# ksahlin/IsoCon

Measured on AMD Instinct MI355X. Metric: read x candidate alignments/sec (NN-graph build, 50k x 2.5kb reads), higher is better.
Workload: dtype u64; 1 GPU; C3: 50000 synthetic CCS reads (50000 unique), ~2500 bp, 10 isoforms, seed 30001; 1-set NN graph; edges=78526, graph_digest=65944c838d76a6c9, parallelism=single GPU

## Files before the change

isocon_amd/csrc/nn_list.hpp:

```cpp
#pragma once
#include "nn.hpp"
#include "nn_surv_core.hpp"

namespace isocon {

static constexpr uint32_t NN_LIST_MIN = 256;
#ifndef ISOCON_NN_LIST_CHUNK
#define ISOCON_NN_LIST_CHUNK 2048
#endif
static constexpr uint32_t NN_LIST_CHUNK = ISOCON_NN_LIST_CHUNK;
static constexpr int NN_STAGE = NN_LIST_CHUNK + 64;
#ifndef ISOCON_SURV_WAVES
#define ISOCON_SURV_WAVES 1
#endif
static constexpr int NN_SURV_WAVES = ISOCON_SURV_WAVES;

struct NNPlanTotals {
    unsigned long long n_pairs, pad0[15], n_list, pad1[15], n_small, pad2[15], n_chunks, pad3[15], n_filtered, pad4[15], overflow, pad5[15];
    unsigned long long n_chunks_narrow, pad6[15];
    unsigned long long n_wide_pairs, n_narrow_listed, pad7[14];
    unsigned long long f_next, pad8[15], f_chunks, pad9[15], f_chunks_narrow, pad10[15], f_rejected, f_narrow_listed, f_listed, f_rejected2, pad11[12];
    unsigned long long f_tasks, pad12[15], f_task_next, pad13[15];
    unsigned long long n_seed_known, pad14[15];
};

static constexpr uint32_t NN_KNOWN_SLOTS = 8;
struct NNSeedKnown { const uint32_t *known; uint32_t drop; };
typedef uint32_t NNKnownRow __attribute__((ext_vector_type(4)));
__device__ __forceinline__ bool nn_seed_known(const uint32_t *__restrict__ known, uint32_t a, uint32_t b)
{
    const NNKnownRow *ra = reinterpret_cast<const NNKnownRow *>(known + (size_t)a * NN_KNOWN_SLOTS), *rb = reinterpret_cast<const NNKnownRow *>(known + (size_t)b * NN_KNOWN_SLOTS);
    const NNKnownRow a0 = ra[0], a1 = ra[1], b0 = rb[0], b1 = rb[1];
    bool hit = false;
#pragma unroll
    for (int i = 0; i < 4; ++i) hit = hit || a0[i] == b || a1[i] == b || b0[i] == a || b1[i] == a;
    return hit;
}

static constexpr int32_t NN_NARROW_K = 31;

struct NNBoundRows {
    const uint8_t *lb;  const unsigned long long *row_off; const uint32_t *row_len;
    const uint8_t *lbT; const unsigned long long *offT;    const uint32_t *sloT; const uint32_t *lenT;
    const uint32_t *score;
};

__device__ __forceinline__ uint32_t nn_meta_len(uint32_t w) { return w & 0x3fffu; }
__device__ __forceinline__ int32_t nn_meta_thr(uint32_t w) { return (int32_t)((w >> 14) & 0x7fu); }
__device__ __forceinline__ uint32_t nn_meta_score(uint32_t w) { return w >> 23; }
static constexpr uint32_t NN_META_PAD = 3;
typedef uint32_t NNMeta4 __attribute__((ext_vector_type(4), aligned(4)));

__global__ __launch_bounds__(256) void k_nn_entry_meta(DevStore S, NNParams P, const uint32_t *__restrict__ score, uint32_t *__restrict__ meta, NNPlanTotals *__restrict__ totals)
{
    const uint32_t x = blockIdx.x * 256u + threadIdx.x;
    if (x >= S.n && x < S.n + NN_META_PAD) meta[x] = 0u;
    if (x < S.n) {
        const int32_t m = S.lens[x], b = load_relaxed_agent(P.best + x);
        int32_t thr = b < m ? b : m;
        thr = thr < 64 ? thr : 64;
        const uint32_t sc = score[x] >> 5;
        const bool isq = P.qflag[x] != 0;
        meta[x] = ((uint32_t)m & 0x3fffu) | ((uint32_t)thr << 14) | ((P.tflag[x] != 0 ? 1u : 0u) << 21) | ((isq ? 1u : 0u) << 22) | ((sc < 511u ? sc : 511u) << 23);
    }
}

__global__ __launch_bounds__(64 * NN_SURV_WAVES) void k_nn_survivors(DevStore S, NNParams P, NNBoundRows B, const uint32_t *__restrict__ meta, QMap Q, uint32_t nq,
                                                       uint32_t *__restrict__ list, unsigned long long list_cap, NNChunk *__restrict__ chunks, unsigned long long chunks_cap,
                                                       uint32_t *__restrict__ pa, uint32_t *__restrict__ pb, unsigned long long small_cap, NNPlanTotals *__restrict__ totals, uint32_t list_min,
                                                       int32_t class_mode, NNSeedKnown K)
{
    __shared__ uint32_t stage[NN_SURV_WAVES][NN_STAGE];
    __shared__ uint32_t s_small[NN_SURV_WAVES], s_filtered[NN_SURV_WAVES], s_kept[NN_SURV_WAVES], s_known[NN_SURV_WAVES];
    __shared__ unsigned long long s_base;
    const int wave = threadIdx.x >> 6;
    const uint32_t x = blockIdx.x * (uint32_t)NN_SURV_WAVES + (uint32_t)wave;
    const int lane = threadIdx.x & 63;
    const uint32_t mx = x < S.n ? meta[x] : 0u;
    const bool x_isq = (mx & (1u << 22)) != 0, x_ist = (mx & (1u << 21)) != 0;
    uint32_t up_len = 0, dn_len = 0, dn_slo = 0;
    unsigned long long up_off = 0, dn_off = 0;
    if (x < S.n && (x_isq || x_ist)) {
        uint32_t s;
        if (Q.slot_of(x, s) && s < nq) {
            up_len = B.row_len[s];
            up_off = B.row_off[s];
        }
        dn_len = B.lenT[x]; dn_slo = B.sloT[x]; dn_off = B.offT[x];
    }
    const int32_t m = (int32_t)nn_meta_len(mx);
    const int32_t kx0 = nn_meta_thr(mx);
    const uint32_t sx = nn_meta_score(mx);
    uint32_t *st = stage[wave];
    uint32_t fill = 0, fill_n = 0, filtered = 0, kept = 0;
    auto emit_chunk = [&](bool narrow_class, bool merged = false) {
        const uint32_t cnt = merged ? fill + fill_n : narrow_class ? fill_n : fill;
        unsigned long long base = 0, ci = 0;
        if (lane == 0) {
            base = atomicAdd(&totals->n_list, (unsigned long long)cnt);
            ci = atomicAdd(narrow_class ? &totals->n_chunks_narrow : &totals->n_chunks, 1ull);
            if (narrow_class) atomicAdd(&totals->n_narrow_listed, (unsigned long long)cnt);
        }
        base = ((unsigned long long)(uint32_t)__builtin_amdgcn_readfirstlane((int)(base >> 32)) << 32) | (uint32_t)__builtin_amdgcn_readfirstlane((int)(uint32_t)base);
        ci = ((unsigned long long)(uint32_t)__builtin_amdgcn_readfirstlane((int)(ci >> 32)) << 32) | (uint32_t)__builtin_amdgcn_readfirstlane((int)(uint32_t)ci);
        if (base + cnt <= list_cap && ci < chunks_cap) {
            if (narrow_class) { for (uint32_t i = (uint32_t)lane; i < cnt; i += 64) list[base + i] = st[NN_STAGE - 1 - i]; }
            else { for (uint32_t i = (uint32_t)lane; i < cnt; i += 64) list[base + i] = i < fill ? st[i] : st[NN_STAGE - 1 - (i - fill)]; }
            if (lane == 0) { NNChunk ch; ch.slot = x; ch.count = cnt; ch.begin = base; chunks[(narrow_class ? chunks_cap : 0ull) + ci] = ch; }
        } else if (lane == 0) atomicOr(&totals->overflow, 1ull);
        if (narrow_class || merged) fill_n = 0;
        if (!narrow_class) fill = 0;
    };
#ifndef ISOCON_SURV_U
#define ISOCON_SURV_U 4
#endif
    constexpr int U = ISOCON_SURV_U;
    const uint32_t q_block = Q.block();
    const uint32_t role_mask = (x_isq ? 1u << 21 : 0u) | (x_ist ? 1u << 22 : 0u);
    auto entry_of = [&](uint32_t s) { return Q.begin + (s >> Q.block_log2) * Q.stride + (s & (q_block - 1u)); };
    auto scan_side = [&](auto side_tag) {
        constexpr int side = decltype(side_tag)::value;
        const uint32_t len = side == 0 ? up_len : dn_len;
        const uint8_t *row = side == 0 ? B.lb + up_off : B.lbT + dn_off;
        const uint32_t tail = (len - 1u) & ~3u;
        auto load_batches = [&](uint32_t c0, uint32_t (&lbv)[U], NNMeta4 (&my)[U]) {
#pragma unroll
            for (int u = 0; u < U; ++u) {
                const uint32_t e0 = c0 + (uint32_t)SURV_BATCH * u + 4u * (uint32_t)lane;
                const uint32_t ec = e0 < len ? e0 : tail;
                __builtin_memcpy(&lbv[u], row + ec, 4);
                if (side == 0) my[u] = *reinterpret_cast<const NNMeta4 *>(meta + (x + 1u + ec));
                else {
                    const uint32_t s0 = dn_slo + ec;
                    const bool apart = Q.stride != q_block && (s0 & (q_block - 1u)) + 3u >= q_block;
                    if (__builtin_amdgcn_ballot_w64(apart) == 0) my[u] = *reinterpret_cast<const NNMeta4 *>(meta + entry_of(s0));
                    else {
#pragma unroll
                        for (int b = 0; b < SURV_PER_LANE; ++b) my[u][b] = meta[entry_of(dn_slo + (ec + b < len ? ec + b : len - 1u))];
                    }
                }
            }
        };
        auto scan_batches = [&](uint32_t c0, const uint32_t (&lbv)[U], const NNMeta4 (&my)[U]) {
#pragma unroll
            for (int u = 0; u < U; ++u) {
                if (c0 + (uint32_t)SURV_BATCH * u >= len) break;
                const uint32_t e0 = c0 + (uint32_t)SURV_BATCH * u + 4u * (uint32_t)lane;
                uint64_t am[SURV_PER_LANE], an[SURV_PER_LANE], aw[SURV_PER_LANE];
#pragma unroll
                for (int b = 0; b < SURV_PER_LANE; ++b) {
                    const uint32_t myb = my[u][b];
                    const bool inr = e0 + b < len;
                    const bool xq = inr && x_isq && (myb & (1u << 21));
                    const bool yq = inr && x_ist && (myb & (1u << 22));
                    int32_t kx = -1, ky = -1;
                    if (xq) kx = kx0;
                    if (yq) ky = nn_meta_thr(myb);
                    int32_t k = kx > ky ? kx : ky;
                    if (k > P.kcap) k = P.kcap;
                    const int32_t dl = m - (int32_t)nn_meta_len(myb), ad = dl < 0 ? -dl : dl;
                    const uint32_t sy_u = nn_meta_score(myb);
                    const bool cand = inr && k >= 0 && ad <= k;
                    const bool accept = cand && (int32_t)((lbv[u] >> (8 * b)) & 0xffu) <= k;
                    const bool mine = accept && (side == 0 ? sy_u <= sx : sx > sy_u);
                    if (side == 0) { filtered += cand && !accept ? 1u : 0u; kept += accept ? 1u : 0u; }
                    const bool wide = mine && class_mode > 0 && k > NN_NARROW_K;
                    const bool keep = mine && !wide;
                    const bool to_narrow = keep && class_mode >= 0 && k <= NN_NARROW_K;
                    aw[b] = __builtin_amdgcn_ballot_w64(wide);
                    am[b] = __builtin_amdgcn_ballot_w64(keep && !to_narrow);
                    an[b] = __builtin_amdgcn_ballot_w64(to_narrow);
                }
                const auto word = [&](int b) {
                    const uint32_t y = side == 0 ? x + 1u + e0 + (uint32_t)b : entry_of(dn_slo + e0 + (uint32_t)b);
                    return y | (my[u][b] & role_mask) << 9;
                };
                if (class_mode > 0) {
                    const uint32_t cw = surv_count(aw, ~(uint64_t)0);
                    if (cw != 0) {
                        unsigned long long wbase = 0;
                        if (lane == 0) {
                            wbase = atomicAdd(&totals->n_small, (unsigned long long)cw);
                            atomicAdd(&totals->n_wide_pairs, (unsigned long long)cw);
                            if (wbase + cw > small_cap) { atomicOr(&totals->overflow, 1ull); wbase = ~0ull; }
                        }
                        wbase = ((unsigned long long)(uint32_t)__builtin_amdgcn_readfirstlane((int)(wbase >> 32)) << 32) | (uint32_t)__builtin_amdgcn_readfirstlane((int)(uint32_t)wbase);
                        if (wbase != ~0ull) {
                            unsigned long long at = wbase + surv_rank(aw, lane);
#pragma unroll
                            for (int b = 0; b < SURV_PER_LANE; ++b) {
                                const uint32_t kw = surv_lane_bit(aw[b], lane);
                                if (kw) { pa[at] = x; pb[at] = word(b) & 0x3fffffffu; }
                                at += kw;
                            }
                        }
                    }
                }
                fill = (uint32_t)__builtin_amdgcn_readfirstlane((int)fill);
                fill_n = (uint32_t)__builtin_amdgcn_readfirstlane((int)fill_n);
                surv_batch(am, an, fill, fill_n, NN_LIST_CHUNK,
                           [&](uint64_t lanes, uint32_t off_a, uint32_t off_n) {
                               if (surv_lane_bit(lanes, lane) == 0) return;
                               uint32_t at_a = off_a + surv_rank(am, lane), at_n = (uint32_t)NN_STAGE - 1u - (off_n + surv_rank(an, lane));
#pragma unroll
                               for (int b = 0; b < SURV_PER_LANE; ++b) {
                                   const uint32_t ka = surv_lane_bit(am[b], lane), kn = surv_lane_bit(an[b], lane);
                                   if (ka | kn) st[ka ? at_a : at_n] = word(b);
                                   at_a += ka;
                                   at_n -= kn;
                               }
                           },
                           [&](bool narrow_class) { emit_chunk(narrow_class); });
            }
        };
        for (uint32_t c0 = 0; c0 < len; c0 += SURV_BATCH * U) {
            uint32_t lbv[U];
            NNMeta4 my[U];
            load_batches(c0, lbv, my);
            scan_batches(c0, lbv, my);
        }
    };
    scan_side(std::integral_constant<int, 0>());
    scan_side(std::integral_constant<int, 1>());
    if (fill_n >= list_min) emit_chunk(true);
    if (fill + fill_n >= list_min) emit_chunk(false, true);
    const uint32_t rest = fill + fill_n;
#pragma unroll
    for (int o = 32; o > 0; o >>= 1) { filtered += __shfl_xor(filtered, o, 64); kept += __shfl_xor(kept, o, 64); }
    static_assert(NN_STAGE <= 64 * 64, "one mask bit per round of the staged pairs");
    const auto item = [&](uint32_t i) { return (i < fill ? st[i] : st[NN_STAGE - 1 - (i - fill)]) & 0x3fffffffu; };
    uint64_t settled_rounds = 0;
    uint32_t n_known = 0;
    if (K.known != nullptr) {
        for (uint32_t i0 = 0, t = 0; i0 < rest; i0 += 64, ++t) {
            const uint32_t i = i0 + (uint32_t)lane;
            const bool settled = i < rest && nn_seed_known(K.known, x, item(i));
            n_known += (uint32_t)__popcll(__builtin_amdgcn_ballot_w64(settled));
            if (settled) settled_rounds |= (uint64_t)1 << t;
        }
    }
    const uint32_t n_out = K.drop ? rest - n_known : rest;
    if (lane == 0) { s_small[wave] = n_out; s_filtered[wave] = filtered; s_kept[wave] = kept; s_known[wave] = n_known; }
    __syncthreads();
    if (threadIdx.x == 0) {
        uint32_t tot = 0, fsum = 0, ksum = 0, nsum = 0;
        for (int w = 0; w < NN_SURV_WAVES; ++w) { tot += s_small[w]; fsum += s_filtered[w]; ksum += s_kept[w]; nsum += s_known[w]; }
        unsigned long long base = 0;
        if (tot) {
            base = atomicAdd(&totals->n_small, (unsigned long long)tot);
            if (base + tot > small_cap) { atomicOr(&totals->overflow, 1ull); base = ~0ull; }
        }
        s_base = base;
        if (fsum) atomicAdd(&totals->n_filtered, (unsigned long long)fsum);
        if (ksum) atomicAdd(&totals->n_pairs, (unsigned long long)ksum);
        if (nsum) atomicAdd(&totals->n_seed_known, (unsigned long long)nsum);
    }
    __syncthreads();
    if (n_out && s_base != ~0ull) {
        unsigned long long base = s_base;
        for (int w = 0; w < wave; ++w) base += s_small[w];
        if (n_out == rest) { for (uint32_t i = (uint32_t)lane; i < rest; i += 64) { pa[base + i] = x; pb[base + i] = item(i); } }
        else {
            const uint64_t below = ((uint64_t)1 << lane) - 1;
            for (uint32_t i0 = 0, t = 0; i0 < rest; i0 += 64, ++t) {
                const uint32_t i = i0 + (uint32_t)lane;
                const bool stays = i < rest && ((settled_rounds >> t) & 1u) == 0;
                const uint64_t sm = __builtin_amdgcn_ballot_w64(stays);
                if (stays) { const unsigned long long at = base + (unsigned long long)__popcll(sm & below); pa[at] = x; pb[at] = item(i); }
                base += (unsigned long long)__popcll(sm);
            }
        }
    }
}

__global__ __launch_bounds__(1024) void k_nn_sort_chunks(const NNChunk *__restrict__ in, uint32_t n, NNChunk *__restrict__ out)
{
    __shared__ uint32_t hist[16], cursor[16];
    if (threadIdx.x < 16) hist[threadIdx.x] = 0;
    __syncthreads();
    auto cls = [](uint32_t count) { const uint32_t c = count / (NN_LIST_CHUNK / 16 + 1); return 15u - (c < 15u ? c : 15u); };
    for (uint32_t i = threadIdx.x; i < n; i += 1024) atomicAdd(&hist[cls(in[i].count)], 1u);
    __syncthreads();
    if (threadIdx.x == 0) { uint32_t a = 0; for (int b = 0; b < 16; ++b) { cursor[b] = a; a += hist[b]; } }
    __syncthreads();
    for (uint32_t i = threadIdx.x; i < n; i += 1024) { const NNChunk c = in[i]; out[atomicAdd(&cursor[cls(c.count)], 1u)] = c; }
}

}
```

isocon_amd/csrc/nn_lists.inc:

```

namespace {

int NNContext::plan_lists(const QMap &Q, uint32_t nq, const NNParams &PR, ListPlan &L)
{
    L = ListPlan();
    if (PR.lb == nullptr || nq == 0 || variant("nn_no_list") || st->pool.slots[SLOT_NN_LBT].p == nullptr || st->maxlen >= 16384) return ISOCON_OK;
    unsigned long long pairs_cap = std::min<unsigned long long>(lb_total, std::max<unsigned long long>(1ull << 22, lb_total / 8));
    if (const char *e = variant_value("nn_list_cap")) pairs_cap = std::max<unsigned long long>(1, strtoull(e, nullptr, 10));
    const bool filter = !variant("nn_no_block_filter") && ensure_text2();
    uint32_t list_min = NN_LIST_MIN;
    if (const char *e = variant_value("nn_list_min")) list_min = (uint32_t)std::max(1, atoi(e));
    const uint32_t build_min = filter ? std::min<uint32_t>(list_min, NNF_LIST_MIN) : list_min;
    const unsigned long long cap_in = pairs_cap / build_min + 1, cap_out = filter ? pairs_cap / list_min + 1 : cap_in;
    size_t free_b = 0;
    if (!free_mem(free_b) || pairs_cap * 12 > free_b / 2 + st->pool.slots[SLOT_NN_LIST].cap * 3) return ISOCON_OK;
    DevBuf *bufs[] = {&d_ltot, &d_lchunks, &d_list, &d_lpa, &d_lpb, &d_lmeta, &d_ltasks};
    const int slots[] = {SLOT_NN_LTOT, SLOT_NN_LCHUNKS, SLOT_NN_LIST, SLOT_NN_LPA, SLOT_NN_LPB, SLOT_NN_LDEST, SLOT_NN_LTASKS};
    for (int i = 0; i < 7; ++i) { bufs[i]->pool = &st->pool; bufs[i]->slot = slots[i]; }
    const bool second = filter && !variant("nn_filter_one_pass");
    const unsigned long long tasks_cap = second ? 2 * cap_in + pairs_cap / 64 + 1 : 0;
    if (second && d_ltasks.alloc((size_t)tasks_cap * sizeof(NNFTask))) return ISOCON_OK;
    const size_t n_records = (size_t)(filter ? 2 * cap_in : 0) + 4 * (size_t)cap_out;
    if (d_lmeta.alloc(((size_t)n + NN_META_PAD) * 4) || d_ltot.alloc(sizeof(NNPlanTotals)) || d_lchunks.alloc(n_records * sizeof(NNChunk)) || d_list.alloc((size_t)pairs_cap * 4) ||
        d_lpa.alloc((size_t)pairs_cap * 4) || d_lpb.alloc((size_t)pairs_cap * 4))
        return ISOCON_OK;
    NNChunk *built = d_lchunks.as<NNChunk>();
    L.a = built + (filter ? 2 * cap_in : 0);
    L.b = L.a + cap_out;
    L.sorted_a = L.b + cap_out;
    L.sorted_b = L.sorted_a + cap_out;
    ISO_HIP_CHECK(hipMemsetAsync(d_ltot.p, 0, sizeof(NNPlanTotals), 0));
    NNBoundRows B;
    B.lb = PR.lb; B.row_off = PR.lb_row; B.row_len = lb_len_dev;
    B.lbT = static_cast<const uint8_t *>(st->pool.slots[SLOT_NN_LBT].p);
    B.offT = static_cast<const unsigned long long *>(st->pool.slots[SLOT_NN_LBT_OFF].p);
    B.sloT = static_cast<const uint32_t *>(st->pool.slots[SLOT_NN_LBT_SLO].p);
    B.lenT = static_cast<const uint32_t *>(st->pool.slots[SLOT_NN_LBT_LEN].p);
    B.score = static_cast<const uint32_t *>(st->pool.slots[SLOT_NN_SCORE].p);
    const NNSeedKnown K = seed_known();
    tm.start();
    int32_t class_mode = 0;
    if (const char *e = variant_value("nn_narrow")) class_mode = atoi(e) > 0 ? 1 : -1;
    hipLaunchKernelGGL(k_nn_entry_meta, dim3((n + NN_META_PAD + 255) / 256), dim3(256), 0, 0, st->dev, PR, B.score, d_lmeta.as<uint32_t>(), d_ltot.as<NNPlanTotals>());
    ISO_HIP_CHECK(hipGetLastError());
    hipLaunchKernelGGL(k_nn_survivors, dim3((n + NN_SURV_WAVES - 1) / NN_SURV_WAVES), dim3(64 * NN_SURV_WAVES), 0, 0, st->dev, PR, B, d_lmeta.as<uint32_t>(), Q, nq, d_list.as<uint32_t>(), pairs_cap,
                       filter ? built : L.a, cap_in, d_lpa.as<uint32_t>(), d_lpb.as<uint32_t>(), pairs_cap, d_ltot.as<NNPlanTotals>(), build_min, class_mode, K);
    ISO_HIP_CHECK(hipGetLastError());
    if (filter) {
        tm.mark();
        ISO_HIP_CHECK(nnf_launch_filter(d_text2.as<uint32_t>(), text2_stride, st->dev.lens, d_lmeta.as<uint32_t>(), PR.kcap, d_list.as<uint32_t>(), built, cap_in, L.a, cap_out,
                                        d_lpa.as<uint32_t>(), d_lpb.as<uint32_t>(), pairs_cap, d_ltot.as<NNPlanTotals>(), list_min,
                                        second ? d_ltasks.as<NNFTask>() : (NNFTask *)nullptr, tasks_cap, K));
    }
    tm.stop_later(&stats.list_kernel_ms, &stats.filter_kernel_ms);
    NNPlanTotals tot;
    ISO_HIP_CHECK(memcpy_wait(&tot, d_ltot.p, sizeof(tot), hipMemcpyDeviceToHost));
    if (tot.overflow) return ISOCON_OK;
    stats.pairs_prefiltered += tot.n_filtered;
    stats.pairs_block_rejected += tot.f_rejected + tot.f_rejected2;
    L.listed = true;
    L.n_chunks = filter ? tot.f_chunks : tot.n_chunks;
    L.n_chunks_narrow = filter ? tot.f_chunks_narrow : tot.n_chunks_narrow;
    L.n_small = tot.n_small;
    L.seed_known = tot.n_seed_known;
    L.K = K;
    stats.pairs_wide_to_lanes += tot.n_wide_pairs;
    unsigned long long table_chunks = NNF_TABLE_CHUNKS;
    if (const char *e = variant_value("nn_table_chunks")) table_chunks = strtoull(e, nullptr, 10);
    if (filter && L.n_chunks + L.n_chunks_narrow > 0 && L.n_chunks + L.n_chunks_narrow < table_chunks) {
        if (tot.n_small + tot.f_listed > pairs_cap) return ISOCON_OK;
        L.conv_a = L.n_chunks; L.conv_b = L.n_chunks_narrow; L.conv_pairs = tot.f_listed;
        L.n_chunks = L.n_chunks_narrow = 0;
        return ISOCON_OK;
    }
    stats.pairs_narrow += filter ? tot.f_narrow_listed : tot.n_narrow_listed;
    return ISOCON_OK;
}

}
```

isocon_amd/csrc/nn_surv_core.hpp:

```cpp
#pragma once
#include "band_core.hpp"

namespace isocon {

static constexpr int SURV_PER_LANE = 4;
static constexpr int SURV_GROUPS = 4;
static constexpr int SURV_BATCH = 64 * SURV_PER_LANE;

ISO_HD uint64_t surv_group_lanes(int j) { return (uint64_t)0xffffu << (16 * j); }

ISO_HD uint32_t surv_count(const uint64_t (&m)[SURV_PER_LANE], uint64_t lanes)
{
    uint32_t c = 0;
#if defined(__HIP_DEVICE_COMPILE__)
#pragma unroll
#endif
    for (int b = 0; b < SURV_PER_LANE; ++b) c += (uint32_t)popc64(m[b] & lanes);
    return c;
}

ISO_HD uint32_t surv_rank(const uint64_t (&m)[SURV_PER_LANE], int lane)
{
    uint32_t r = 0;
#if defined(__HIP_DEVICE_COMPILE__)
    (void)lane;
#pragma unroll
    for (int b = 0; b < SURV_PER_LANE; ++b) r = __builtin_amdgcn_mbcnt_hi((uint32_t)(m[b] >> 32), __builtin_amdgcn_mbcnt_lo((uint32_t)m[b], r));
#else
    const uint64_t below = ((uint64_t)1 << lane) - 1;
    for (int b = 0; b < SURV_PER_LANE; ++b) r += (uint32_t)popc64(m[b] & below);
#endif
    return r;
}

ISO_HD uint32_t surv_lane_bit(uint64_t m, int lane)
{
#if defined(__HIP_DEVICE_COMPILE__)
    (void)lane;
    uint32_t r;
    asm("v_cndmask_b32_e64 %0, 0, 1, %1" : "=v"(r) : "s"(m));
    return r;
#else
    return (uint32_t)(m >> lane) & 1u;
#endif
}


template <class Write, class Flush>
ISO_HD void surv_batch(const uint64_t (&am)[SURV_PER_LANE], const uint64_t (&an)[SURV_PER_LANE], uint32_t &fill, uint32_t &fill_n, uint32_t chunk, Write write, Flush flush)
{
    const uint32_t ca = surv_count(am, ~(uint64_t)0), cn = surv_count(an, ~(uint64_t)0);
    if (ca + cn == 0) return;
    if (fill + fill_n + ca + cn < chunk) {
        write(~(uint64_t)0, fill, fill_n);
        fill += ca;
        fill_n += cn;
        return;
    }
    uint32_t before_a = 0, before_n = 0;
#if defined(__HIP_DEVICE_COMPILE__)
#pragma unroll 1
#endif
    for (int j = 0; j < SURV_GROUPS; ++j) {
        const uint64_t lanes = surv_group_lanes(j);
        const uint32_t ga = surv_count(am, lanes), gn = surv_count(an, lanes);
        if (ga + gn != 0) {
            write(lanes, fill - before_a, fill_n - before_n);
            fill += ga;
            fill_n += gn;
            if (fill + fill_n >= chunk) flush(fill_n > fill);
        }
        before_a += ga;
        before_n += gn;
    }
}

}
```

Before: 83.16 billion alignments/s.

## Add packed SWAR survivor test with byte-packed side metadata arrays

Adds side arrays (role byte, 7-bit length byte, 16-bit score) written by the meta kernel, and a templated packed survivor kernel path. It tests four candidates per lane at once using SIMD-within-a-register byte arithmetic instead of per-element scalar compares. It also splits full and tail iterations and skips staging when no lane keeps anything. The aim is lower per-candidate ALU and memory traffic in the survivor scan. The cost is more metadata writes, extra memory, and a truncated length-difference test whose correctness depends on kcap<=63.

Measured after the change: 84.64 billion alignments/s, median of 6. +1.8%, better.

```diff
diff --git a/isocon_amd/csrc/nn_list.hpp b/isocon_amd/csrc/nn_list.hpp
--- a/isocon_amd/csrc/nn_list.hpp
+++ b/isocon_amd/csrc/nn_list.hpp
@@ -51,21 +51,46 @@
 static constexpr uint32_t NN_META_PAD = 3;
 typedef uint32_t NNMeta4 __attribute__((ext_vector_type(4), aligned(4)));
 
-__global__ __launch_bounds__(256) void k_nn_entry_meta(DevStore S, NNParams P, const uint32_t *__restrict__ score, uint32_t *__restrict__ meta, NNPlanTotals *__restrict__ totals)
+struct NNSurvSide {
+    const uint8_t *role, *len7;
+    const uint16_t *score;
+};
+static inline bool nn_surv_packed(int32_t kcap, int32_t class_mode) { return class_mode <= 0 && kcap >= 0 && kcap <= 63; }
+static inline size_t nn_meta_bytes(size_t n) { return (n + NN_META_PAD) * 8; }
+static inline NNSurvSide nn_surv_side(uint32_t *meta, size_t n)
+{
+    NNSurvSide s;
+    uint16_t *sc = reinterpret_cast<uint16_t *>(meta + (n + NN_META_PAD));
+    uint8_t *role = reinterpret_cast<uint8_t *>(sc + (n + NN_META_PAD));
+    s.score = sc; s.role = role; s.len7 = role + (n + NN_META_PAD);
+    return s;
+}
+
+__global__ __launch_bounds__(256) void k_nn_entry_meta(DevStore S, NNParams P, const uint32_t *__restrict__ score, uint32_t *__restrict__ meta, NNSurvSide A, NNPlanTotals *__restrict__ totals)
 {
     const uint32_t x = blockIdx.x * 256u + threadIdx.x;
-    if (x >= S.n && x < S.n + NN_META_PAD) meta[x] = 0u;
+    if (x >= S.n && x < S.n + NN_META_PAD) {
+        meta[x] = 0u;
+        const_cast<uint8_t *>(A.role)[x] = 0;
+        const_cast<uint8_t *>(A.len7)[x] = surv_len_byte(0);
+        const_cast<uint16_t *>(A.score)[x] = surv_score_half(0);
+    }
     if (x < S.n) {
         const int32_t m = S.lens[x], b = load_relaxed_agent(P.best + x);
         int32_t thr = b < m ? b : m;
         thr = thr < 64 ? thr : 64;
         const uint32_t sc = score[x] >> 5;
-        const bool isq = P.qflag[x] != 0;
-        meta[x] = ((uint32_t)m & 0x3fffu) | ((uint32_t)thr << 14) | ((P.tflag[x] != 0 ? 1u : 0u) << 21) | ((isq ? 1u : 0u) << 22) | ((sc < 511u ? sc : 511u) << 23);
-    }
-}
-
-__global__ __launch_bounds__(64 * NN_SURV_WAVES) void k_nn_survivors(DevStore S, NNParams P, NNBoundRows B, const uint32_t *__restrict__ meta, QMap Q, uint32_t nq,
+        const bool isq = P.qflag[x] != 0, ist = P.tflag[x] != 0;
+        const uint32_t sc9 = sc < 511u ? sc : 511u;
+        meta[x] = ((uint32_t)m & 0x3fffu) | ((uint32_t)thr << 14) | ((ist ? 1u : 0u) << 21) | ((isq ? 1u : 0u) << 22) | (sc9 << 23);
+        const_cast<uint8_t *>(A.role)[x] = surv_role_byte(ist, isq, thr, P.kcap);
+        const_cast<uint8_t *>(A.len7)[x] = surv_len_byte((uint32_t)m);
+        const_cast<uint16_t *>(A.score)[x] = surv_score_half(sc9);
+    }
+}
+
+template <bool PACKED>
+__global__ __launch_bounds__(64 * NN_SURV_WAVES) void k_nn_survivors(DevStore S, NNParams P, NNBoundRows B, const uint32_t *__restrict__ meta, NNSurvSide A, QMap Q, uint32_t nq,
                                                        uint32_t *__restrict__ list, unsigned long long list_cap, NNChunk *__restrict__ chunks, unsigned long long chunks_cap,
                                                        uint32_t *__restrict__ pa, uint32_t *__restrict__ pb, unsigned long long small_cap, NNPlanTotals *__restrict__ totals, uint32_t list_min,
                                                        int32_t class_mode, NNSeedKnown K)
@@ -87,6 +112,12 @@
             up_off = B.row_off[s];
         }
         dn_len = B.lenT[x]; dn_slo = B.sloT[x]; dn_off = B.offT[x];
+    }
+    if constexpr (PACKED && NN_SURV_WAVES == 1) {
+        const auto uni = [](uint32_t v) { return (uint32_t)__builtin_amdgcn_readfirstlane((int)v); };
+        up_len = uni(up_len); dn_len = uni(dn_len); dn_slo = uni(dn_slo);
+        up_off = ((unsigned long long)uni((uint32_t)(up_off >> 32)) << 32) | uni((uint32_t)up_off);
+        dn_off = ((unsigned long long)uni((uint32_t)(dn_off >> 32)) << 32) | uni((uint32_t)dn_off);
     }
     const int32_t m = (int32_t)nn_meta_len(mx);
     const int32_t kx0 = nn_meta_thr(mx);
@@ -118,6 +149,23 @@
     const uint32_t q_block = Q.block();
     const uint32_t role_mask = (x_isq ? 1u << 21 : 0u) | (x_ist ? 1u << 22 : 0u);
     auto entry_of = [&](uint32_t s) { return Q.begin + (s >> Q.block_log2) * Q.stride + (s & (q_block - 1u)); };
+    auto stage_batch = [&](const uint64_t (&am)[SURV_PER_LANE], const uint64_t (&an)[SURV_PER_LANE], auto word) {
+        fill = (uint32_t)__builtin_amdgcn_readfirstlane((int)fill);
+        fill_n = (uint32_t)__builtin_amdgcn_readfirstlane((int)fill_n);
+        surv_batch(am, an, fill, fill_n, NN_LIST_CHUNK,
+                   [&](uint64_t lanes, uint32_t off_a, uint32_t off_n) {
+                       if (surv_lane_bit(lanes, lane) == 0) return;
+                       uint32_t at_a = off_a + surv_rank(am, lane), at_n = (uint32_t)NN_STAGE - 1u - (off_n + surv_rank(an, lane));
+#pragma unroll
+                       for (int b = 0; b < SURV_PER_LANE; ++b) {
+                           const uint32_t ka = surv_lane_bit(am[b], lane), kn = surv_lane_bit(an[b], lane);
+                           if (ka | kn) st[ka ? at_a : at_n] = word(b);
+                           at_a += ka;
+                           at_n -= kn;
+                       }
+                   },
+                   [&](bool narrow_class) { emit_chunk(narrow_class); });
+    };
     auto scan_side = [&](auto side_tag) {
         constexpr int side = decltype(side_tag)::value;
         const uint32_t len = side == 0 ? up_len : dn_len;
@@ -150,26 +198,12 @@
 #pragma unroll
                 for (int b = 0; b < SURV_PER_LANE; ++b) {
                     const uint32_t myb = my[u][b];
-                    const bool inr = e0 + b < len;
-                    const bool xq = inr && x_isq && (myb & (1u << 21));
-                    const bool yq = inr && x_ist && (myb & (1u << 22));
-                    int32_t kx = -1, ky = -1;
-                    if (xq) kx = kx0;
-                    if (yq) ky = nn_meta_thr(myb);
-                    int32_t k = kx > ky ? kx : ky;
-                    if (k > P.kcap) k = P.kcap;
-                    const int32_t dl = m - (int32_t)nn_meta_len(myb), ad = dl < 0 ? -dl : dl;
-                    const uint32_t sy_u = nn_meta_score(myb);
-                    const bool cand = inr && k >= 0 && ad <= k;
-                    const bool accept = cand && (int32_t)((lbv[u] >> (8 * b)) & 0xffu) <= k;
-                    const bool mine = accept && (side == 0 ? sy_u <= sx : sx > sy_u);
-                    if (side == 0) { filtered += cand && !accept ? 1u : 0u; kept += accept ? 1u : 0u; }
-                    const bool wide = mine && class_mode > 0 && k > NN_NARROW_K;
-                    const bool keep = mine && !wide;
-                    const bool to_narrow = keep && class_mode >= 0 && k <= NN_NARROW_K;
-                    aw[b] = __builtin_amdgcn_ballot_w64(wide);
-                    am[b] = __builtin_amdgcn_ballot_w64(keep && !to_narrow);
-                    an[b] = __builtin_amdgcn_ballot_w64(to_narrow);
+                    const SurvTest t = surv_test(e0 + b < len, x_isq, x_ist, (myb & (1u << 22)) != 0, (myb & (1u << 21)) != 0, kx0, nn_meta_thr(myb), P.kcap, m, (int32_t)nn_meta_len(myb),
+                                                 (lbv[u] >> (8 * b)) & 0xffu, sx, nn_meta_score(myb), side, class_mode);
+                    if (side == 0) { filtered += t.cand && !t.accept ? 1u : 0u; kept += t.accept ? 1u : 0u; }
+                    aw[b] = __builtin_amdgcn_ballot_w64(t.wide);
+                    am[b] = __builtin_amdgcn_ballot_w64(t.keep && !t.to_narrow);
+                    an[b] = __builtin_amdgcn_ballot_w64(t.to_narrow);
                 }
                 const auto word = [&](int b) {
                     const uint32_t y = side == 0 ? x + 1u + e0 + (uint32_t)b : entry_of(dn_slo + e0 + (uint32_t)b);
@@ -196,21 +230,7 @@
                         }
                     }
                 }
-                fill = (uint32_t)__builtin_amdgcn_readfirstlane((int)fill);
-                fill_n = (uint32_t)__builtin_amdgcn_readfirstlane((int)fill_n);
-                surv_batch(am, an, fill, fill_n, NN_LIST_CHUNK,
-                           [&](uint64_t lanes, uint32_t off_a, uint32_t off_n) {
-                               if (surv_lane_bit(lanes, lane) == 0) return;
-                               uint32_t at_a = off_a + surv_rank(am, lane), at_n = (uint32_t)NN_STAGE - 1u - (off_n + surv_rank(an, lane));
-#pragma unroll
-                               for (int b = 0; b < SURV_PER_LANE; ++b) {
-                                   const uint32_t ka = surv_lane_bit(am[b], lane), kn = surv_lane_bit(an[b], lane);
-                                   if (ka | kn) st[ka ? at_a : at_n] = word(b);
-                                   at_a += ka;
-                                   at_n -= kn;
-                               }
-                           },
-                           [&](bool narrow_class) { emit_chunk(narrow_class); });
+                stage_batch(am, an, word);
             }
         };
         for (uint32_t c0 = 0; c0 < len; c0 += SURV_BATCH * U) {
@@ -220,8 +240,88 @@
             scan_batches(c0, lbv, my);
         }
     };
-    scan_side(std::integral_constant<int, 0>());
-    scan_side(std::integral_constant<int, 1>());
+    uint32_t ncand_p = 0, kept_p = 0;
+    auto scan_side_packed = [&](auto side_tag) {
+        constexpr int side = decltype(side_tag)::value;
+        const uint32_t len = side == 0 ? up_len : dn_len;
+        const uint8_t *row = side == 0 ? B.lb + up_off : B.lbT + dn_off;
+        const uint32_t tail = (len - 1u) & ~3u;
+        const SurvX X = surv_x(x_isq, x_ist, kx0, P.kcap, m, sx, side, class_mode);
+        const bool blocks_apart = side != 0 && Q.stride != q_block;
+        auto iteration = [&](uint32_t c0, auto full_tag) {
+            constexpr bool full = decltype(full_tag)::value;
+            uint32_t lbv[U], role[U], len7[U];
+            uint2 sc[U];
+#pragma unroll
+            for (int u = 0; u < U; ++u) {
+                const uint32_t e0 = c0 + (uint32_t)SURV_BATCH * u + 4u * (uint32_t)lane;
+                const uint32_t ec = full || e0 < len ? e0 : tail;
+                __builtin_memcpy(&lbv[u], row + ec, 4);
+                const uint32_t y0 = side == 0 ? x + 1u + ec : entry_of(dn_slo + ec);
+                const bool apart = blocks_apart && ((dn_slo + ec) & (q_block - 1u)) + 3u >= q_block;
+                if (!blocks_apart || __builtin_amdgcn_ballot_w64(apart) == 0) {
+                    __builtin_memcpy(&role[u], A.role + y0, 4);
+                    __builtin_memcpy(&len7[u], A.len7 + y0, 4);
+                    __builtin_memcpy(&sc[u], A.score + y0, 8);
+                } else {
+                    role[u] = len7[u] = 0u;
+                    sc[u] = make_uint2(0u, 0u);
+#pragma unroll
+                    for (int b = 0; b < SURV_PER_LANE; ++b) {
+                        const uint32_t y = entry_of(dn_slo + (ec + b < len ? ec + b : len - 1u));
+                        role[u] |= (uint32_t)A.role[y] << (8 * b);
+                        len7[u] |= (uint32_t)A.len7[y] << (8 * b);
+                        if (b < 2) sc[u].x |= (uint32_t)A.score[y] << (16 * b);
+                        else sc[u].y |= (uint32_t)A.score[y] << (16 * (b - 2));
+                    }
+                }
+            }
+            uint32_t keep[U], any = 0u;
+#pragma unroll
+            for (int u = 0; u < U; ++u) {
+                const uint32_t e0 = c0 + (uint32_t)SURV_BATCH * u + 4u * (uint32_t)lane;
+                if (!full) role[u] &= surv_inr_bytes((int32_t)len - (int32_t)e0);
+                uint32_t cand, accept;
+                surv_test4<side>(X, lbv[u], role[u], len7[u], sc[u].x, sc[u].y, cand, accept, keep[u]);
+                if (side == 0) { ncand_p += (uint32_t)__popc(cand); kept_p += (uint32_t)__popc(accept); }
+                any |= keep[u];
+            }
+            if (__builtin_amdgcn_ballot_w64(any != 0u) == 0) return;
+#pragma unroll 1
+            for (int u = 0; u < U; ++u) {
+                uint32_t keep_u = keep[0], role_u = role[0];
+#pragma unroll
+                for (int v = 1; v < U; ++v) { keep_u = u == v ? keep[v] : keep_u; role_u = u == v ? role[v] : role_u; }
+                if (__builtin_amdgcn_ballot_w64(keep_u != 0u) == 0) continue;
+                const uint32_t e0 = c0 + (uint32_t)SURV_BATCH * (uint32_t)u + 4u * (uint32_t)lane;
+                const uint32_t kn = keep_u & surv_narrow4(X, role_u), ka = keep_u & ~kn;
+                uint64_t am[SURV_PER_LANE], an[SURV_PER_LANE];
+#pragma unroll
+                for (int b = 0; b < SURV_PER_LANE; ++b) {
+                    am[b] = __builtin_amdgcn_ballot_w64((ka & (0x80u << (8 * b))) != 0u);
+                    an[b] = __builtin_amdgcn_ballot_w64((kn & (0x80u << (8 * b))) != 0u);
+                }
+                const auto word = [&](int b) {
+                    const uint32_t y = side == 0 ? x + 1u + e0 + (uint32_t)b : entry_of(dn_slo + e0 + (uint32_t)b);
+                    const uint32_t rb = role_u >> (8 * b);
+                    return y | (x_isq && (rb & 0x80u) ? 1u << 30 : 0u) | (x_ist && (rb & 0x7fu) ? 1u << 31 : 0u);
+                };
+                stage_batch(am, an, word);
+            }
+        };
+        uint32_t c0 = 0;
+        for (; c0 + (uint32_t)(SURV_BATCH * U) <= len; c0 += SURV_BATCH * U) iteration(c0, std::true_type());
+        if (c0 < len) iteration(c0, std::false_type());
+    };
+    if constexpr (PACKED) {
+        scan_side_packed(std::integral_constant<int, 0>());
+        scan_side_packed(std::integral_constant<int, 1>());
+        filtered += ncand_p - kept_p;
+        kept += kept_p;
+    } else {
+        scan_side(std::integral_constant<int, 0>());
+        scan_side(std::integral_constant<int, 1>());
+    }
     if (fill_n >= list_min) emit_chunk(true);
     if (fill + fill_n >= list_min) emit_chunk(false, true);
     const uint32_t rest = fill + fill_n;
diff --git a/isocon_amd/csrc/nn_lists.inc b/isocon_amd/csrc/nn_lists.inc
--- a/isocon_amd/csrc/nn_lists.inc
+++ b/isocon_amd/csrc/nn_lists.inc
@@ -21,7 +21,7 @@
     const unsigned long long tasks_cap = second ? 2 * cap_in + pairs_cap / 64 + 1 : 0;
     if (second && d_ltasks.alloc((size_t)tasks_cap * sizeof(NNFTask))) return ISOCON_OK;
     const size_t n_records = (size_t)(filter ? 2 * cap_in : 0) + 4 * (size_t)cap_out;
-    if (d_lmeta.alloc(((size_t)n + NN_META_PAD) * 4) || d_ltot.alloc(sizeof(NNPlanTotals)) || d_lchunks.alloc(n_records * sizeof(NNChunk)) || d_list.alloc((size_t)pairs_cap * 4) ||
+    if (d_lmeta.alloc(nn_meta_bytes(n)) || d_ltot.alloc(sizeof(NNPlanTotals)) || d_lchunks.alloc(n_records * sizeof(NNChunk)) || d_list.alloc((size_t)pairs_cap * 4) ||
         d_lpa.alloc((size_t)pairs_cap * 4) || d_lpb.alloc((size_t)pairs_cap * 4))
         return ISOCON_OK;
     NNChunk *built = d_lchunks.as<NNChunk>();
@@ -41,9 +41,11 @@
     tm.start();
     int32_t class_mode = 0;
     if (const char *e = variant_value("nn_narrow")) class_mode = atoi(e) > 0 ? 1 : -1;
-    hipLaunchKernelGGL(k_nn_entry_meta, dim3((n + NN_META_PAD + 255) / 256), dim3(256), 0, 0, st->dev, PR, B.score, d_lmeta.as<uint32_t>(), d_ltot.as<NNPlanTotals>());
+    const NNSurvSide side = nn_surv_side(d_lmeta.as<uint32_t>(), n);
+    auto *const survivors = nn_surv_packed(PR.kcap, class_mode) && !variant("nn_surv_scalar") ? k_nn_survivors<true> : k_nn_survivors<false>;
+    hipLaunchKernelGGL(k_nn_entry_meta, dim3((n + NN_META_PAD + 255) / 256), dim3(256), 0, 0, st->dev, PR, B.score, d_lmeta.as<uint32_t>(), side, d_ltot.as<NNPlanTotals>());
     ISO_HIP_CHECK(hipGetLastError());
-    hipLaunchKernelGGL(k_nn_survivors, dim3((n + NN_SURV_WAVES - 1) / NN_SURV_WAVES), dim3(64 * NN_SURV_WAVES), 0, 0, st->dev, PR, B, d_lmeta.as<uint32_t>(), Q, nq, d_list.as<uint32_t>(), pairs_cap,
+    hipLaunchKernelGGL(survivors, dim3((n + NN_SURV_WAVES - 1) / NN_SURV_WAVES), dim3(64 * NN_SURV_WAVES), 0, 0, st->dev, PR, B, d_lmeta.as<uint32_t>(), side, Q, nq, d_list.as<uint32_t>(), pairs_cap,
                        filter ? built : L.a, cap_in, d_lpa.as<uint32_t>(), d_lpb.as<uint32_t>(), pairs_cap, d_ltot.as<NNPlanTotals>(), build_min, class_mode, K);
     ISO_HIP_CHECK(hipGetLastError());
     if (filter) {
diff --git a/isocon_amd/csrc/nn_surv_core.hpp b/isocon_amd/csrc/nn_surv_core.hpp
--- a/isocon_amd/csrc/nn_surv_core.hpp
+++ b/isocon_amd/csrc/nn_surv_core.hpp
@@ -45,6 +45,88 @@
 #endif
 }
 
+struct SurvTest { bool cand, accept, mine, wide, keep, to_narrow; };
+static constexpr int32_t SURV_NARROW_K = 31;
+
+ISO_HD SurvTest surv_test(bool inr, bool x_isq, bool x_ist, bool y_isq, bool y_ist, int32_t kx0, int32_t thr_y, int32_t kcap, int32_t m, int32_t len_y, uint32_t bound,
+                          uint32_t sx, uint32_t sy, int side, int32_t class_mode)
+{
+    SurvTest t;
+    const bool xq = inr && x_isq && y_ist;
+    const bool yq = inr && x_ist && y_isq;
+    int32_t kx = -1, ky = -1;
+    if (xq) kx = kx0;
+    if (yq) ky = thr_y;
+    int32_t k = kx > ky ? kx : ky;
+    if (k > kcap) k = kcap;
+    const int32_t dl = m - len_y, ad = dl < 0 ? -dl : dl;
+    t.cand = inr && k >= 0 && ad <= k;
+    t.accept = t.cand && (int32_t)bound <= k;
+    t.mine = t.accept && (side == 0 ? sy <= sx : sx > sy);
+    t.wide = t.mine && class_mode > 0 && k > SURV_NARROW_K;
+    t.keep = t.mine && !t.wide;
+    t.to_narrow = t.keep && class_mode >= 0 && k <= SURV_NARROW_K;
+    return t;
+}
+
+static constexpr uint32_t SURV_H = 0x80808080u;
+ISO_HD uint8_t surv_role_byte(bool is_t, bool is_q, int32_t thr, int32_t kcap)
+{
+    const int32_t c = kcap < 63 ? (kcap < 0 ? 0 : kcap) : 63, k = thr < c ? thr : c;
+    return (uint8_t)((is_t ? 0x80u : 0u) | (is_q ? (uint32_t)(k < 0 ? 0 : k) + 1u : 0u));
+}
+ISO_HD uint8_t surv_len_byte(uint32_t len) { return (uint8_t)(0x80u | (len & 0x7fu)); }
+ISO_HD uint16_t surv_score_half(uint32_t score) { return (uint16_t)(0x8000u | (score & 0x1ffu)); }
+
+struct SurvX {
+    uint32_t a4;
+    uint32_t bm;
+    uint32_t m4;
+    uint32_t s2;
+    uint32_t nb;
+    uint32_t ua;
+    uint32_t cm;
+};
+ISO_HD SurvX surv_x(bool x_isq, bool x_ist, int32_t kx0, int32_t kcap, int32_t m, uint32_t sx, int side, int32_t class_mode)
+{
+    SurvX X;
+    const uint32_t a = x_isq ? (uint32_t)(kx0 < kcap ? kx0 : kcap) + 1u : 0u;
+    X.a4 = a * 0x01010101u;
+    X.bm = x_ist ? 0x7f7f7f7fu : 0u;
+    X.m4 = (((uint32_t)m & 0x7fu) + (side == 0 ? 0u : 1u)) * 0x01010101u;
+    X.s2 = (sx + (side == 0 ? 1u : 0u)) * 0x00010001u;
+    X.nb = x_ist ? 0x21212121u : SURV_H;
+    X.ua = a > (uint32_t)SURV_NARROW_K + 1u ? SURV_H : 0u;
+    X.cm = class_mode >= 0 ? SURV_H : 0u;
+    return X;
+}
+
+ISO_HD uint32_t surv_inr_bytes(int32_t n) { return n <= 0 ? 0u : n >= 4 ? ~0u : (1u << (8 * n)) - 1u; }
+
+ISO_HD uint32_t surv_odd_bytes(uint32_t lo, uint32_t hi)
+{
+#if defined(__HIP_DEVICE_COMPILE__)
+    return __builtin_amdgcn_perm(hi, lo, 0x07050301u);
+#else
+    return ((lo >> 8) & 0xffu) | ((lo >> 16) & 0xff00u) | ((hi << 8) & 0xff0000u) | (hi & 0xff000000u);
+#endif
+}
+
+template <int SIDE>
+ISO_HD void surv_test4(const SurvX &X, uint32_t bound, uint32_t role, uint32_t len7, uint32_t s01, uint32_t s23, uint32_t &cand, uint32_t &accept, uint32_t &keep)
+{
+    const uint32_t d0 = len7 - X.m4;
+    const uint32_t d = (SIDE == 0 ? d0 : ~d0) | SURV_H;
+    const uint32_t b4 = role & X.bm;
+    const uint32_t e = bound | SURV_H;
+    const uint32_t c1 = (~(d - X.a4) & role) | ~(d - b4);
+    const uint32_t c2 = (~(e - X.a4) & role) | ~(e - b4);
+    cand = c1 & SURV_H;
+    accept = cand & c2 & ~bound;
+    keep = accept & ~surv_odd_bytes(s01 - X.s2, s23 - X.s2);
+}
+ISO_HD uint32_t surv_narrow4(const SurvX &X, uint32_t role) { return ~(((role | SURV_H) - X.nb) | (role & X.ua)) & X.cm; }
+
 
 template <class Write, class Flush>
 ISO_HD void surv_batch(const uint64_t (&am)[SURV_PER_LANE], const uint64_t (&an)[SURV_PER_LANE], uint32_t &fill, uint32_t &fill_n, uint32_t chunk, Write write, Flush flush)
```
